# adria0/plonk-by-fingers

Measured on AMD Instinct MI355X. Metric: NTT elements/sec (Goldilocks, n=2^20 per GPU, natural order, bit-exact vs src/fft.rs), higher is better.
Workload: dtype u64 (Goldilocks p=2^64-2^32+1); 1 GPU; Goldilocks forward NTT, batch 32 x 2^20; n_per_gpu=1048576, n_global=1048576, batch=32, passes=default (2^20: 10,10)

## Files before the change

plonk-by-fingers_amd/csrc/internal.hpp:

```cpp
#pragma once
#include <hip/hip_runtime.h>
#include <stdint.h>
#include <cstdlib>
#include <map>
#include <memory>
#include <string>
#include <tuple>
#include <vector>
#include "field.hpp"

struct pbf_ctx;

namespace pbf {

typedef unsigned __int128 u128;
static const uint64_t GOLDILOCKS = 0xFFFFFFFF00000001ull;

enum FieldKind { FIELD_GOLDILOCKS = 0, FIELD_MOD32 = 1 };

void set_error(const std::string& s);

struct Options {
  std::map<std::string, std::string> kv;
  const char* get(const char* name) const {
    auto it = kv.find(name);
    return it == kv.end() ? nullptr : it->second.c_str();
  }
  long long num(const char* name, long long dflt) const {
    const char* v = get(name);
    return v && *v ? atoll(v) : dflt;
  }
};

int fail(int code, const std::string& s);

#define PBF_HIP(expr)                                                                        \
  do {                                                                                       \
    hipError_t e_ = (expr);                                                                  \
    if (e_ != hipSuccess)                                                                    \
      return ::pbf::fail(3 , std::string(#expr) + ": " + hipGetErrorString(e_)); \
  } while (0)

inline uint64_t hmul(uint64_t a, uint64_t b, uint64_t m) { return (uint64_t)(((u128)a * b) % m); }
inline uint64_t hpow(uint64_t a, uint64_t e, uint64_t m) {
  uint64_t r = 1 % m;
  while (e) {
    if (e & 1) r = hmul(r, a, m);
    a = hmul(a, a, m);
    e >>= 1;
  }
  return r;
}
bool hinv(uint64_t a, uint64_t m, uint64_t* out);

bool field_for(uint64_t m, FieldKind* kind, FieldArgs* fa);

struct DevBuf {
  void* p = nullptr;
  size_t bytes = 0;
  int ensure(size_t need);
  void release();
  ~DevBuf();
};

struct CosetTabs {
  uint64_t shift = 0, len = 0, stamp = 0;
  uint32_t bits = 0;
  DevBuf t0, t1;
  DevBuf tc_last;
};
constexpr size_t COSET_SHIFTS_PER_PLAN = 4;

struct NttPlan {
  uint64_t m = 0, omega = 0, n = 0;
  int inverse = 0;
  uint64_t root = 0;
  FieldKind kind = FIELD_GOLDILOCKS;
  FieldArgs fa{};
  uint32_t log_n = 0;
  uint64_t n_inv = 1;
  Options opts;
  std::vector<int> logr;
  int e64 = -1;
  std::vector<std::shared_ptr<DevBuf>> twpass;
  uint32_t tw_bits = 0;
  DevBuf tw0, tw1, small_tw;
  int twmax_log = 24;
  bool gl = false;
  std::vector<std::shared_ptr<DevBuf>> rtab;
  std::vector<std::shared_ptr<DevBuf>> tc;
  std::shared_ptr<DevBuf> tws_a, tws_b;
  int tws_w = 0;
  bool rg = false;
  mutable bool rg_built = false;
  mutable DevBuf rg_tc1, rg_t2;
  mutable DevBuf rg_tgc, rg_tgb;
  mutable std::vector<std::unique_ptr<CosetTabs>> coset;
  mutable uint64_t coset_clock = 0;
};

constexpr int GL_MAX_STREAMS = 8;
struct ForkSet {
  int device = 0;
  hipStream_t aux[GL_MAX_STREAMS] = {};
  hipEvent_t fork = nullptr, join[GL_MAX_STREAMS] = {};
  int ensure(int streams);
  ~ForkSet();
};

constexpr int MSM_TAIL_SLOTS = 3;
struct MsmTail {
  int device = 0;
  hipStream_t aux = nullptr;
  hipEvent_t ready[MSM_TAIL_SLOTS] = {}, done[MSM_TAIL_SLOTS] = {};
  bool used[MSM_TAIL_SLOTS] = {};
  int next = 0, last = -1;
  int ensure();
  ~MsmTail();
};

int make_plan(uint64_t m, uint64_t omega, uint64_t n, int inverse, NttPlan* p);
int run_plan(const NttPlan& p, const uint64_t* d_in, uint64_t* d_out, size_t batch, DevBuf& s0, DevBuf& s1,
             hipStream_t stream, ForkSet* fork = nullptr);
int run_plan_coset(const NttPlan& p, uint64_t shift, const uint64_t* d_in, size_t in_len, uint64_t* d_out,
                   size_t batch, DevBuf& s0, DevBuf& s1, hipStream_t stream, ForkSet* fork = nullptr);
int launch_pointwise_mul(FieldKind k, const FieldArgs& fa, const uint64_t* a, const uint64_t* b, uint64_t* c,
                         uint64_t count, hipStream_t s);
int launch_poly_eval(FieldKind k, const FieldArgs& fa, const uint64_t* d_coeffs, uint64_t n, const uint64_t* d_xs,
                     uint64_t nx, uint64_t* d_ys, DevBuf& partial, hipStream_t s);
struct TwoLevel {
  DevBuf t0, t1;
  uint64_t root = 0;
  uint32_t bits = 0;
};
int make_two_level(uint64_t m, uint64_t root, uint64_t n, TwoLevel* t);
int run_plan_split(const NttPlan& p, const uint64_t* d_in, uint64_t* d_send, size_t batch, uint32_t G, DevBuf& s0,
                   DevBuf& s1, DevBuf& s2, hipStream_t stream);
int launch_shard_combine(FieldKind k, const FieldArgs& fa, const TwoLevel& tl, uint32_t G, uint64_t rank,
                         const uint64_t* in, uint64_t* out, uint64_t nl, uint32_t batch, int inverse, hipStream_t s);
int launch_shard_unsplit(const uint64_t* recv, uint64_t* out, uint64_t nl, uint32_t batch, uint32_t G,
                         hipStream_t s);
int launch_fill_random(const FieldArgs& fa, FieldKind k, uint64_t seed, uint64_t* d_out, uint64_t count,
                       hipStream_t s);

int pairing_check_on_stream(pbf_ctx* ctx, const uint64_t* g1, const uint64_t* g2, size_t n, int* ok, hipStream_t s);

}

struct pbf_ctx {
  int device = 0;
  pbf::Options options;
  uint64_t serial = 0;
  hipStream_t stream = nullptr;
  hipStream_t user_stream = nullptr;
  std::map<std::tuple<uint64_t, uint64_t, uint64_t, int>, std::unique_ptr<pbf::NttPlan>> plans;
  pbf::DevBuf scratch0, scratch1, scratch2, io0, io1, io2, partial;
  pbf::ForkSet fork;
  struct FixedBase {
    bool valid = false;
    uint64_t n = 0;
    int c = 16;
    pbf::DevBuf table;
    pbf::DevBuf inf;
  } fixed_base;
  std::map<std::tuple<uint64_t, uint64_t, uint64_t>, std::unique_ptr<pbf::TwoLevel>> two_level;
  int roots(uint64_t m, uint64_t root, uint64_t n, pbf::TwoLevel** out);
  static hipStream_t pick(void* s) { return (hipStream_t)s; }
  hipStream_t host_stream() const { return user_stream ? user_stream : stream; }
  int plan(uint64_t m, uint64_t omega, uint64_t n, int inverse, pbf::NttPlan** out);
  std::map<std::string, std::unique_ptr<pbf::DevBuf>> named;
  pbf::DevBuf& buf(const std::string& name) {
    auto& b = named[name];
    if (!b) b.reset(new pbf::DevBuf());
    return *b;
  }
// ... 9 lines not shown
```

plonk-by-fingers_amd/csrc/ntt_gl.hpp:

```cpp
#pragma once
#include "ntt_kernels.hpp"

namespace pbf {

struct GlPassArgs {
  const uint64_t* in;
  uint64_t* out;
  const uint64_t* twpass;
  const uint64_t* tw0;
  const uint64_t* tw1;
  const uint64_t* tc;
  const uint64_t* tws_a;
  const uint64_t* tws_b;
  uint64_t n;
  uint32_t log_n;
  uint32_t log_ns;
  uint32_t tw_bits;
  uint32_t blocks_per_poly;
  uint32_t batch;
  uint32_t scaled;
  uint32_t out_split_log;
  uint32_t xcd_kmajor;
  uint64_t in_pitch, out_pitch;
  const uint64_t* post_tw;
  uint32_t skip_pass_tw;
  const uint64_t* cs_tab;
  const uint64_t* cs_tab1;
  uint32_t cs_bits;
  uint64_t cs_len;
};

__host__ __device__ constexpr bool gl_pow2_neg(int k) {
  const int raw = ((k % 192) + 192) % 192;
  return raw > 64 && raw <= 160;
}
template <int K>
__device__ __forceinline__ uint64_t gl_pow2_abs(uint64_t x) {
  constexpr int RAW = ((K % 192) + 192) % 192;
  if constexpr (RAW == 0) {
    return x;
  } else if constexpr (RAW > 160) {
    return gl_div_pow2<192 - RAW>(x);
  } else {
    using T = ShiftKind<RAW>;
    static_assert(T::NEG == gl_pow2_neg(K), "sign of 2^K");
    return apply_shift<Goldilocks, T>(x);
  }
}
template <int K>
__device__ __forceinline__ uint64_t gl_pow2(uint64_t x) {
  const uint64_t y = gl_pow2_abs<K>(x);
  if constexpr (gl_pow2_neg(K)) {
    const FieldArgs f{};
    return Goldilocks::sub(0, y, f);
  } else {
    return y;
  }
}

template <int E64, int Q1, int S2 = 1>
__device__ __forceinline__ void gl_stage_b_twiddle(uint64_t* v) {
  if constexpr (S2 < 16) {
    v[S2] = gl_pow2<(E64 * S2 * Q1) % 192>(v[S2]);
    gl_stage_b_twiddle<E64, Q1, S2 + 1>(v);
  }
}
template <int E64, int Q1, int S2 = 1>
__device__ __forceinline__ void gl_stage_b_twiddle_abs(uint64_t* v) {
  if constexpr (S2 < 16) {
    v[S2] = gl_pow2_abs<(E64 * S2 * Q1) % 192>(v[S2]);
    gl_stage_b_twiddle_abs<E64, Q1, S2 + 1>(v);
  }
}
__host__ __device__ constexpr unsigned gl_stage_b_negmask(int e64, int q1) {
  unsigned m = 0;
  for (int s2 = 1; s2 < 16; ++s2) m |= gl_pow2_neg((e64 * s2 * q1) % 192) ? 1u << s2 : 0u;
  return m;
}
constexpr int GL_B_LEVELS = 2;
template <int E64, int Q1>
__device__ __forceinline__ void gl_stage_b_head(uint64_t* v) {
  const FieldArgs f{};
  gl_stage_b_twiddle_abs<E64, Q1>(v);
  dft_reg_signed<Goldilocks, 4, sub_root_exp(E64, 4), gl_stage_b_negmask(E64, Q1), GL_B_LEVELS>(v, f);
}

template <int E64, int Q, int E = 1>
__device__ __forceinline__ void gl_post_twiddle_br(uint64_t* v) {
  if constexpr (E < 16) {
    v[bitrev_c(E, 4)] = gl_pow2<(E64 * E * Q) % 192>(v[bitrev_c(E, 4)]);
    gl_post_twiddle_br<E64, Q, E + 1>(v);
  }
}
template <int E64, int WV, int U = 0>
__device__ __forceinline__ void gl_rg3_c_shift(uint64_t* x) {
  if constexpr (U < 4) {
    constexpr int g = WV + 4 * U;
    x[U * 4 + 1] = gl_pow2<(E64 * g) % 192>(x[U * 4 + 1]);
    x[U * 4 + 2] = gl_pow2<(E64 * 2 * g) % 192>(x[U * 4 + 2]);
    x[U * 4 + 3] = gl_pow2<(E64 * 3 * g) % 192>(x[U * 4 + 3]);
    gl_rg3_c_shift<E64, WV, U + 1>(x);
  }
}

template <int LOGR, int TILE>
struct GlShape {
  static constexpr int R = 1 << LOGR;
  static constexpr int LOGC = LOGR - 6;
  static constexpr int C = 1 << LOGC;
  static constexpr int W = TILE / R;
  static constexpr int NT = TILE / 16;
  static constexpr int WPQ = NT / 256;
  static constexpr bool YX = W == 16 && C > 1;
  static constexpr int YP = (YX ? 64 : 65) * W;
  static constexpr int LDS = (C * YP > TILE) ? C * YP : TILE;
  static constexpr bool LDS32K = LDS * 8 <= 32768;
  static constexpr int NSUB_C = (64 * W) / NT;
  __host__ __device__ static constexpr int ysw(int k1) {
    return W <= 32 ? (k1 / (32 / W)) & (W - 1) : (k1 & 31);
  }
  __host__ __device__ static constexpr int yidx(int r2, int k1, int w) {
    return r2 * YP + (YX ? (k1 ^ (r2 & 1)) : k1) * W + (w ^ ysw(k1));
  }
};

__device__ __forceinline__ void gl_tile_coords(const GlPassArgs& a, uint32_t tile, uint32_t tiles, uint32_t* poly,
                                               uint32_t* kb) {
  if (a.xcd_kmajor == 1) {
    const uint32_t v = (tile & 7) * (tiles >> 3) + (tile >> 3);
    *kb = v / a.batch;
    *poly = v % a.batch;
  } else if (a.xcd_kmajor == 2) {
    const uint32_t v = (tile & 7) * (tiles >> 3) + (tile >> 3);
    *poly = v / a.blocks_per_poly;
    *kb = v % a.blocks_per_poly;
  } else {
    *poly = tile / a.blocks_per_poly;
    *kb = tile % a.blocks_per_poly;
  }
}

__device__ __forceinline__ uint64_t gl_cs_factor(const GlPassArgs& a, uint64_t i) {
  const FieldArgs f{};
  if (a.cs_tab1) return Goldilocks::mul(a.cs_tab[i & ((1ull << a.cs_bits) - 1)], a.cs_tab1[i >> a.cs_bits], f);
  return a.cs_tab[i];
}

constexpr int GL_STORES = 16;

template <int LOGR, int E64, bool FIRST, int TILE, int RG = 0, int CS = 0, int SP = 0>
__device__ __forceinline__ void gl_tile(const GlPassArgs& a, uint64_t* lds, uint32_t tile, uint32_t tiles, int t) {
  using Sh = GlShape<LOGR, TILE>;
  constexpr int C = Sh::C, LOGC = Sh::LOGC, W = Sh::W, NT = Sh::NT, YP = Sh::YP;
  (void)YP;
  static_assert(Sh::NSUB_C * C == GL_STORES, "stores per thread");
  static_assert(SP == 0 || (!FIRST && RG == 0 && CS == 0 && SP <= 2), "SP: second pass of a plain two-pass plan");
  static_assert(RG == 0 || (LOGR == 8 && TILE == 4096 && FIRST == (RG == 1)), "RG shape");
  static_assert(CS == 0 || (FIRST == (CS == 1) && (RG == 0 || RG == 2 * CS - 1)), "CS 1: first pass, CS 2: last pass");
  const FieldArgs f{};
  using G = Goldilocks;
  uint32_t poly, kb;
  gl_tile_coords(a, tile, tiles, &poly, &kb);
  const uint64_t j0 = (uint64_t)kb * W;
  const uint64_t* in = a.in + (uint64_t)poly * a.in_pitch;
  const uint64_t stride = a.n >> LOGR;

  uint64_t v[16];
  if constexpr (CS == 1) {
#pragma unroll
    for (int h = 0; h < 2; ++h) {
      uint64_t tw[8];
#pragma unroll
      for (int uu = 0; uu < 2; ++uu) {
        const int idx = t + NT * (2 * h + uu);
        const int w = idx % W, r2 = (idx / W) % C, s2 = idx / (C * W);
#pragma unroll
        for (int s1 = 0; s1 < 4; ++s1) {
          const uint64_t i = (j0 + w) + (uint64_t)(16 * C * s1 + C * s2 + r2) * stride;
          const bool on = i < a.cs_len;
          v[8 * h + uu * 4 + s1] = on ? in[i] : 0;
          tw[uu * 4 + s1] = on ? gl_cs_factor(a, i) : 0;
        }
      }
#pragma unroll
      for (int m = 0; m < 8; ++m) v[8 * h + m] = G::mul(v[8 * h + m], tw[m], f);
    }
  } else {
#pragma unroll
    for (int u = 0; u < 4; ++u) {
      const int idx = t + NT * u;
      const int w = idx % W, r2 = (idx / W) % C, s2 = idx / (C * W);
#pragma unroll
      for (int s1 = 0; s1 < 4; ++s1) {
        const int r = 16 * C * s1 + C * s2 + r2;
        v[u * 4 + s1] = in[(j0 + w) + (uint64_t)r * stride];
      }
    }
  }
  uint64_t t3[RG == 3 ? 2 : 1];
  if constexpr (RG == 3) {
    const int wave = t >> 6, q1 = wave / Sh::WPQ, rw = (wave % Sh::WPQ) * 64 + (t & 63);
    const int r2 = rw / W, w = rw % W;
    const uint64_t X = ((uint64_t)q1 << 16) + j0 + w;
    t3[0] = a.tws_a[((uint64_t)r2 << 18) + X];
    t3[1] = a.tws_b[X];
  }
  if constexpr (!FIRST && RG != 3 && SP == 0) if (!a.skip_pass_tw) {
    const uint64_t kmask = (1ull << a.log_ns) - 1;
#pragma unroll
    for (int h = 0; h < 2; ++h) {
      uint64_t tw[8];
#pragma unroll
      for (int uu = 0; uu < 2; ++uu) {
        const int u = 2 * h + uu;
        const int idx = t + NT * u;
        const int w = idx % W, r2 = (idx / W) % C, s2 = idx / (C * W);
        const uint64_t k = (j0 + w) & kmask;
#pragma unroll
        for (int s1 = 0; s1 < 4; ++s1) {
          const uint64_t r = (uint64_t)(16 * C * s1 + C * s2 + r2);
          if (a.twpass) {
            tw[uu * 4 + s1] = a.twpass[(r << a.log_ns) + k];
          } else if (a.tws_a) {
            tw[uu * 4 + s1] = G::mul(a.tws_b[(uint64_t)kb * Sh::R + r], a.tws_a[r * W + w], f);
          } else {
            const uint64_t e = ((r * k) << (a.log_n - a.log_ns - LOGR)) & (a.n - 1);
            tw[uu * 4 + s1] = G::mul(a.tw0[e & ((1ull << a.tw_bits) - 1)], a.tw1[e >> a.tw_bits], f);
          }
        }
      }
#pragma unroll
      for (int m = 0; m < 8; ++m) v[8 * h + m] = G::mul(v[8 * h + m], tw[m], f);
    }
  }
#pragma unroll
  for (int u = 0; u < 4; ++u) dft_reg<G, 2, sub_root_exp(E64, 2)>(v + u * 4, nullptr, f);
#pragma unroll
  for (int u = 0; u < 4; ++u) {
    const int idx = t + NT * u;
    const int s2 = idx / (C * W), rw = idx % (C * W);
#pragma unroll
    for (int q1 = 0; q1 < 4; ++q1) lds[(q1 * 16 + s2) * (C * W) + rw] = v[u * 4 + bitrev_c(q1, 2)];
  }
  __syncthreads();

  {
    const int wave = t >> 6;
    const int q1 = wave / Sh::WPQ;
    const int rw = (wave % Sh::WPQ) * 64 + (t & 63);
#pragma unroll
    for (int s2 = 0; s2 < 16; ++s2) v[s2] = lds[(q1 * 16 + s2) * (C * W) + rw];
    if constexpr (RG == 3) {
      uint64_t p = t3[0];
      const uint64_t d = t3[1];
#pragma unroll
      for (int s2 = 0; s2 < 16; ++s2) {
        v[s2] = G::mul(v[s2], p, f);
        if (s2 < 15) p = G::mul(p, d, f);
      }
      dft_reg<G, 4, sub_root_exp(E64, 4)>(v, nullptr, f);
    } else {
      switch (__builtin_amdgcn_readfirstlane(q1)) {
        case 1: gl_stage_b_head<E64, 1>(v); break;
        case 2: gl_stage_b_head<E64, 2>(v); break;
        case 3: gl_stage_b_head<E64, 3>(v); break;
        default: gl_stage_b_head<E64, 0>(v); break;
      }
      dft_reg_tail<G, 4, sub_root_exp(E64, 4), GL_B_LEVELS>(v, f);
    }
    __syncthreads();
    const int r2 = rw / W, w = rw % W;
#pragma unroll
    for (int q2 = 0; q2 < 16; ++q2) {
      const int k1 = q1 + 4 * q2;
      lds[Sh::yidx(r2, k1, w)] = v[bitrev_c(q2, 4)];
    }
  }
  __syncthreads();

  auto c_map = [&](int u, int* k1, int* w) {
    const int idx = t + NT * u;
    if constexpr (FIRST) {
      *k1 = idx & 63;
      *w = idx >> 6;
    } else {
      *k1 = idx / W;
      *w = idx % W;
    }
  };
  uint64_t x[Sh::NSUB_C * C];
#pragma unroll
  for (int u = 0; u < Sh::NSUB_C; ++u) {
    int k1, w;
    c_map(u, &k1, &w);
#pragma unroll
    for (int r2 = 0; r2 < C; ++r2) x[u * C + r2] = lds[Sh::yidx(r2, k1, w)];
  }
  if constexpr (RG == 3) {
    switch (__builtin_amdgcn_readfirstlane(t >> 6)) {
      case 0: gl_rg3_c_shift<E64, 0>(x); break;
      case 1: gl_rg3_c_shift<E64, 1>(x); break;
      case 2: gl_rg3_c_shift<E64, 2>(x); break;
      default: gl_rg3_c_shift<E64, 3>(x); break;
    }
  } else if constexpr (RG == 1) {
    const uint64_t* tc = a.tc + ((j0 >> 12) & 15) * 256;
#pragma unroll
    for (int u = 0; u < Sh::NSUB_C; ++u) {
      int k1, w;
      c_map(u, &k1, &w);
      uint64_t tw[C];
#pragma unroll
      for (int r2 = 0; r2 < C; ++r2) tw[r2] = tc[r2 * 64 + k1];
#pragma unroll
      for (int r2 = 0; r2 < C; ++r2) x[u * C + r2] = G::mul(x[u * C + r2], tw[r2], f);
    }
  } else {
    uint64_t tw[Sh::NSUB_C * C];
    const bool scaled = SP == 0 && a.scaled;
    const int r2lo = scaled ? 0 : 1;
#pragma unroll
    for (int u = 0; u < Sh::NSUB_C; ++u) {
      int k1, w;
      c_map(u, &k1, &w);
#pragma unroll
      for (int r2 = 0; r2 < C; ++r2) tw[u * C + r2] = (r2 >= r2lo) ? a.tc[r2 * 64 + k1] : 1;
    }
    if (scaled) {
#pragma unroll
      for (int m = 0; m < Sh::NSUB_C * C; ++m) x[m] = G::mul(x[m], tw[m], f);
    } else {
#pragma unroll
      for (int u = 0; u < Sh::NSUB_C; ++u)
#pragma unroll
        for (int r2 = 1; r2 < C; ++r2) x[u * C + r2] = G::mul(x[u * C + r2], tw[u * C + r2], f);
    }
  }
  if constexpr (C > 1) {
#pragma unroll
    for (int u = 0; u < Sh::NSUB_C; ++u) dft_reg<G, LOGC, sub_root_exp(E64, LOGC)>(x + u * C, nullptr, f);
  }

  if constexpr (FIRST) {
    uint64_t* o = a.out + (uint64_t)poly * a.out_pitch;
#pragma unroll
    for (int u = 0; u < Sh::NSUB_C; ++u) {
      int k1, w;
      c_map(u, &k1, &w);
      const uint64_t base = (j0 + w) << LOGR;
      if (a.post_tw) {
        uint64_t tw[C];
#pragma unroll
        for (int k2 = 0; k2 < C; ++k2) tw[k2] = a.post_tw[base + k1 + 64 * k2];
#pragma unroll
        for (int k2 = 0; k2 < C; ++k2) x[u * C + bitrev_c(k2, LOGC)] = G::mul(x[u * C + bitrev_c(k2, LOGC)], tw[k2], f);
      }
#pragma unroll
      for (int k2 = 0; k2 < C; ++k2) o[base + k1 + 64 * k2] = x[u * C + bitrev_c(k2, LOGC)];
    }
  } else {
    const uint32_t lns = SP == 2 ? (uint32_t)LOGR : a.log_ns;
    const uint64_t ns_mask = (1ull << lns) - 1;
    uint64_t* out = a.out + (uint64_t)poly * a.out_pitch;
    const uint32_t sl = SP != 0 ? 0u : a.out_split_log;
#pragma unroll
    for (int u = 0; u < Sh::NSUB_C; ++u) {
      int k1, w;
      c_map(u, &k1, &w);
      const uint64_t j = j0 + w;
      const uint64_t base = ((j >> lns) << (lns + LOGR)) + (j & ns_mask);
      if (sl == 0) {
        if constexpr (CS == 2) {
          uint64_t tw[C];
#pragma unroll
          for (int k2 = 0; k2 < C; ++k2) tw[k2] = gl_cs_factor(a, base + ((uint64_t)(k1 + 64 * k2) << lns));
#pragma unroll
          for (int k2 = 0; k2 < C; ++k2) x[u * C + bitrev_c(k2, LOGC)] = G::mul(x[u * C + bitrev_c(k2, LOGC)], tw[k2], f);
        }
#pragma unroll
        for (int k2 = 0; k2 < C; ++k2) out[base + ((uint64_t)(k1 + 64 * k2) << lns)] = x[u * C + bitrev_c(k2, LOGC)];
      } else {
        const uint64_t smask = (1ull << sl) - 1;
#pragma unroll
        for (int k2 = 0; k2 < C; ++k2) {
          const uint64_t kk = base + ((uint64_t)(k1 + 64 * k2) << lns);
          a.out[((((kk >> sl) * a.batch) + poly) << sl) + (kk & smask)] = x[u * C + bitrev_c(k2, LOGC)];
        }
      }
    }
  }
}

template <int LOGR, int TILE>
__device__ __forceinline__ void gl_shape_checks() {
  using Sh = GlShape<LOGR, TILE>;
  static_assert(LOGR >= 6 && LOGR <= 10, "radix 2^6 .. 2^10");
  static_assert(Sh::LDS * 8 <= (TILE > 8192 ? 160 : 80) * 1024, "LDS budget");
  static_assert(Sh::W >= 8 && Sh::WPQ >= 1, "tile shape");
}

template <int LOGR, int E64, bool FIRST, int TILE, int RG = 0, int CS = 0, int SP = 0>
__global__ void __launch_bounds__(TILE / 16)
__attribute__((amdgpu_waves_per_eu((FIRST || RG) && GlShape<LOGR, TILE>::LDS32K ? 5 : 4)))
ntt_gl_pass_kernel(GlPassArgs a) {
  gl_shape_checks<LOGR, TILE>();
  __shared__ __attribute__((aligned(16))) uint64_t lds[GlShape<LOGR, TILE>::LDS];
  const uint32_t tiles = a.blocks_per_poly * a.batch;
  gl_tile<LOGR, E64, FIRST, TILE, RG, CS, SP>(a, lds, blockIdx.x, tiles, threadIdx.x);
}

template <int E64>
__global__ void __launch_bounds__(256) __attribute__((amdgpu_waves_per_eu(4))) ntt_gl_rg2_kernel(GlPassArgs a) {
  constexpr int W = 16;
  __shared__ __attribute__((aligned(16))) uint64_t lds[16 * 16 * W];
  const FieldArgs f{};
  using G = Goldilocks;
  const uint32_t tiles = a.blocks_per_poly * a.batch;
  uint32_t poly, kb;
  gl_tile_coords(a, blockIdx.x, tiles, &poly, &kb);
  const int t = threadIdx.x, w = t % W, a1h = t / W;
  const uint64_t j0 = (uint64_t)kb * W, j = j0 + w;
  const uint32_t c = (uint32_t)(j0 >> 6) & 3, a1l = (uint32_t)(j0 >> 14) & 3;
  const uint64_t* in = a.in + (uint64_t)poly * a.in_pitch;
  const uint64_t stride = a.n >> 8;
  uint64_t v[16], tw[16];
#pragma unroll
// ... 32 lines not shown
```

plonk-by-fingers_amd/csrc/ntt_launch.hip:

```cpp
#include <cstdlib>
#include <cstring>
#include <mutex>
#include "internal.hpp"
#include "ntt_gl.hpp"

namespace pbf {

bool hinv(uint64_t a, uint64_t m, uint64_t* out) {
  __int128 s = 0, old_s = 1, r = m, old_r = a % m;
  while (r != 0) {
    __int128 q = old_r / r, t;
    t = old_r - q * r; old_r = r; r = t;
    t = old_s - q * s; old_s = s; s = t;
  }
  if (old_r != 1) return false;
  if (old_s < 0) old_s += m;
  *out = (uint64_t)old_s;
  return true;
}

bool field_for(uint64_t m, FieldKind* kind, FieldArgs* fa) {
  fa->m = m;
  fa->mu = 0;
  if (m == GOLDILOCKS) { *kind = FIELD_GOLDILOCKS; return true; }
  if (m >= 3 && m < (1ull << 32) && (m & 1)) {
    *kind = FIELD_MOD32;
    fa->mu = (uint64_t)(((u128)1 << 64) / m);
    return true;
  }
  return false;
}

int DevBuf::ensure(size_t need) {
  if (need <= bytes) return 0;
  if (p) (void)hipFree(p);
  p = nullptr;
  bytes = 0;
  hipError_t e = hipMalloc(&p, need);
  if (e != hipSuccess) { p = nullptr; return fail(3, std::string("hipMalloc: ") + hipGetErrorString(e)); }
  bytes = need;
  return 0;
}
void DevBuf::release() {
  if (p) (void)hipFree(p);
  p = nullptr;
  bytes = 0;
}
DevBuf::~DevBuf() { release(); }

static int upload(DevBuf& b, const std::vector<uint64_t>& v) {
  int rc = b.ensure(v.size() * 8);
  if (rc) return rc;
  PBF_HIP(hipMemcpy(b.p, v.data(), v.size() * 8, hipMemcpyHostToDevice));
  return 0;
}

typedef std::vector<uint64_t> Table;

static Table geometric(uint64_t c, uint64_t s, uint64_t count, uint64_t m) {
  Table t(count);
  uint64_t x = c % m;
  for (uint64_t i = 0; i < count; ++i) { t[i] = x; x = hmul(x, s, m); }
  return t;
}

static std::pair<Table, Table> two_level_tabs(uint64_t root, uint64_t len, uint32_t bits, uint64_t c, uint64_t m) {
  return {geometric(c, root, 1ull << bits, m),
          geometric(1, hpow(root, 1ull << bits, m), ((len - 1) >> bits) + 1, m)};
}

static Table stage_c_tab(uint64_t w_r, uint64_t C, uint64_t scale, uint64_t m) {
  Table tc(C * 64);
  for (uint64_t r2 = 0; r2 < C; ++r2)
    for (uint64_t k1 = 0; k1 < 64; ++k1) tc[r2 * 64 + k1] = hmul(hpow(w_r, r2 * k1, m), scale, m);
  return tc;
}

static Table pass_tab(uint64_t w_p, uint64_t R, uint64_t ns, uint64_t m) {
  Table t;
  t.reserve(R * ns);
  for (uint64_t r = 0; r < R; ++r) {
    const Table row = geometric(1, hpow(w_p, r, m), ns, m);
    t.insert(t.end(), row.begin(), row.end());
  }
  return t;
}

static std::pair<Table, Table> split_tabs(uint64_t w_p, uint64_t R, uint64_t W, uint64_t ns, uint64_t m) {
  Table ta = pass_tab(w_p, R, W, m), tb((ns / W) * R);
  for (uint64_t r = 0; r < R; ++r) {
    const Table col = geometric(1, hpow(w_p, r * W, m), ns / W, m);
    for (uint64_t kb = 0; kb < ns / W; ++kb) tb[kb * R + r] = col[kb];
  }
  return {ta, tb};
}

static std::vector<int> default_passes(uint32_t log_n, const Options& o) {
  const char* env = o.get("ntt.passes");
  if (env && *env) {
    std::vector<int> v;
    int sum = 0;
    for (const char* c = env; *c;) {
      int x = atoi(c);
      v.push_back(x);
      sum += x;
      while (*c && *c != ',') ++c;
      if (*c == ',') ++c;
    }
    bool ok = sum == (int)log_n;
    for (int x : v) ok = ok && x >= 6 && x <= 12;
    if (ok) return v;
  }
  int p = (log_n + 9) / 10;
  std::vector<int> v(p, log_n / p);
  for (int i = 0; i < (int)(log_n % p); ++i) v[i] += 1;
  return v;
}

static constexpr int gl_tile(int logr) { return logr >= 10 ? 8192 : 4096; }

int make_plan(uint64_t m, uint64_t omega, uint64_t n, int inverse, NttPlan* p) {
  if (!field_for(m, &p->kind, &p->fa)) return fail(5, "unsupported modulus");
  if (n == 0 || (n & (n - 1))) return fail(1, "n must be a power of two");
  if (n > (1ull << 32)) return fail(1, "n too large");
  if (omega >= m) return fail(1, "omega not canonical");
  uint32_t log_n = 0;
  while ((1ull << log_n) < n) ++log_n;
  if (n > 1) {
    if (hpow(omega, n, m) != 1 || hpow(omega, n / 2, m) == 1) return fail(1, "omega does not have order n");
  }
  p->m = m; p->omega = omega; p->n = n; p->inverse = inverse; p->log_n = log_n;
  p->root = omega;
  if (inverse) {
    if (!hinv(n % m, m, &p->n_inv)) return fail(2, "n has no inverse modulo M (fft.rs:73 unwrap)");
    if (!hinv(omega, m, &p->root)) return fail(1, "omega not invertible");
  }
  const uint64_t w = p->root;
  const long long tm = p->opts.num("ntt.twmax_log", 24);
  p->twmax_log = (int)(tm < 0 ? 0 : (tm > 30 ? 30 : tm));
  if (n <= 4096) return upload(p->small_tw, geometric(1, w, n, m));
  p->logr = default_passes(log_n, p->opts);
  p->tw_bits = (log_n + 1) / 2;
  p->e64 = -1;
  if (p->kind == FIELD_GOLDILOCKS) {
    const uint64_t w64 = hpow(w, n / 64, m);
    if (w64 == hpow(2, 39, m)) p->e64 = 39;
    else if (w64 == hpow(2, 153, m)) p->e64 = 153;
  }
  p->gl = p->e64 >= 0;
  for (int lr : p->logr) p->gl = p->gl && lr >= 6 && lr <= 10;
  p->rg = p->gl && log_n == 24 && p->logr == std::vector<int>{8, 8, 8} && p->opts.num("ntt.no_rg", 0) == 0;

  int rc;
  const auto tw = two_level_tabs(w, n, p->tw_bits, 1, m);
  if ((rc = upload(p->tw0, tw.first)) || (rc = upload(p->tw1, tw.second))) return rc;
  const size_t P = p->logr.size();
  uint64_t ns = 1;
  for (size_t i = 0; i < P; ++i) {
    const uint64_t R = 1ull << p->logr[i], w_p = hpow(w, n / (ns * R), m);
    p->twpass.push_back(std::make_shared<DevBuf>());
    if (ns > 1 && R * ns <= (1ull << p->twmax_log) && (rc = upload(*p->twpass[i], pass_tab(w_p, R, ns, m)))) return rc;
    const long long ts = p->opts.num("ntt.twsplit", -1);
    const uint64_t W = (uint64_t)gl_tile(p->logr[i]) >> p->logr[i];
    if (i + 1 == P && ns > 1 && p->e64 >= 0 && ts != 0 && p->logr[i] >= 6 && p->logr[i] <= 10 &&
        (!p->twpass[i]->p || ts == 1) && ns % W == 0) {
      if (ts == 1) p->twpass[i] = std::make_shared<DevBuf>();
      const auto ab = split_tabs(w_p, R, W, ns, m);
      p->tws_a = std::make_shared<DevBuf>();
      p->tws_b = std::make_shared<DevBuf>();
      if ((rc = upload(*p->tws_a, ab.first)) || (rc = upload(*p->tws_b, ab.second))) return rc;
      p->tws_w = (int)W;
    }
    ns *= R;
  }
  for (size_t i = 0; i < P; ++i) {
    const uint64_t R = 1ull << p->logr[i], w_r = hpow(w, n / R, m);
    auto b = std::make_shared<DevBuf>();
    if (p->gl) {
      rc = upload(*b, stage_c_tab(w_r, R / 64, (inverse && i + 1 == P) ? p->n_inv : 1, m));
      p->tc.push_back(b);
    } else {
      rc = upload(*b, geometric(1, w_r, R, m));
      p->rtab.push_back(b);
    }
    if (rc) return rc;
  }
  return 0;
}

template <class Fn>
static auto with_field(FieldKind k, Fn&& fn) {
  return k == FIELD_GOLDILOCKS ? fn(Goldilocks{}) : fn(Mod32{});
}

typedef void (*PassFn)(PassArgs);

static constexpr int cols_for(int logr) {
  return logr < 10 ? 16 : (logr == 10 ? 8 : (logr == 11 ? 8 : 4));
}

template <class F, int E>
static PassFn pass_fn_e(int logr) {
#define PBF_PASS(LR) \
  case LR: return ntt_pass_kernel<F, LR, cols_for(LR), ((cols_for(LR) << LR) >> NTT_LQ), E>;
  switch (logr) {
    PBF_PASS(6) PBF_PASS(7) PBF_PASS(8) PBF_PASS(9) PBF_PASS(10) PBF_PASS(11) PBF_PASS(12)
    default: return nullptr;
  }
#undef PBF_PASS
}

static PassFn pass_fn(FieldKind k, int e64, int logr) {
  if (k == FIELD_MOD32) return pass_fn_e<Mod32, -1>(logr);
  if (e64 == 39) return pass_fn_e<Goldilocks, 39>(logr);
  if (e64 == 153) return pass_fn_e<Goldilocks, 153>(logr);
  return pass_fn_e<Goldilocks, -1>(logr);
}

struct GlCoset {
  const CosetTabs* tabs;
  uint64_t in_len;
};

static int run_plan_impl(const NttPlan& p, const uint64_t* d_in, uint64_t* d_out, size_t batch, DevBuf& s0,
                         DevBuf& s1, hipStream_t stream, uint32_t split_log, ForkSet* fork = nullptr,
                         const GlCoset* cs = nullptr);

int run_plan(const NttPlan& p, const uint64_t* d_in, uint64_t* d_out, size_t batch, DevBuf& s0, DevBuf& s1,
             hipStream_t stream, ForkSet* fork) {
  return run_plan_impl(p, d_in, d_out, batch, s0, s1, stream, 0, fork);
}

__global__ void shard_split_kernel(const uint64_t* in, uint64_t* out, uint64_t s, uint64_t nl, uint32_t batch) {
  const uint64_t total = nl * batch;
  for (uint64_t id = (uint64_t)blockIdx.x * blockDim.x + threadIdx.x; id < total;
       id += (uint64_t)gridDim.x * blockDim.x) {
    const uint64_t b = id / nl, k = id % nl;
    out[((k / s) * batch + b) * s + (k % s)] = in[id];
  }
}

static uint64_t grid_for(uint64_t count) {
  uint64_t b = (count + 255) / 256;
  return b > 8192 ? 8192 : (b ? b : 1);
}

int run_plan_split(const NttPlan& p, const uint64_t* d_in, uint64_t* d_send, size_t batch, uint32_t G, DevBuf& s0,
                   DevBuf& s1, DevBuf& s2, hipStream_t stream) {
  const uint64_t S = p.n / G;
  uint32_t sl = 0;
  while ((1ull << sl) < S) ++sl;
  if (!p.logr.empty() && S >= 16 && p.logr.size() >= 2) return run_plan_impl(p, d_in, d_send, batch, s0, s1, stream, sl);
  int rc = s2.ensure(batch * p.n * 8);
  if (rc) return rc;
  if ((rc = run_plan_impl(p, d_in, (uint64_t*)s2.p, batch, s0, s1, stream, 0))) return rc;
  hipLaunchKernelGGL(shard_split_kernel, dim3(grid_for(p.n * batch)), dim3(256), 0, stream, (const uint64_t*)s2.p,
                     d_send, S, p.n, (uint32_t)batch);
  PBF_HIP(hipGetLastError());
  return 0;
}

int launch_shard_unsplit(const uint64_t* recv, uint64_t* out, uint64_t nl, uint32_t batch, uint32_t G,
                         hipStream_t s) {
  hipLaunchKernelGGL(shard_unsplit_kernel, dim3(grid_for(nl * batch)), dim3(256), 0, s, recv, out, nl / G, nl, batch,
                     G);
  PBF_HIP(hipGetLastError());
  return 0;
}

int make_two_level(uint64_t m, uint64_t root, uint64_t n, TwoLevel* t) {
  uint32_t log_n = 0;
  while ((1ull << log_n) < n) ++log_n;
  t->bits = (log_n + 1) / 2;
  t->root = root;
  const auto tw = two_level_tabs(root, n, t->bits, 1, m);
  int rc = upload(t->t0, tw.first);
  return rc ? rc : upload(t->t1, tw.second);
}

template <class F>
static int combine_typed(const FieldArgs& fa, const TwoLevel& tl, uint32_t G, uint64_t rank, const uint64_t* in,
                         uint64_t* out, uint64_t nl, uint32_t batch, int inverse, hipStream_t s) {
  CombineArgs a;
  a.recv = in; a.out = out;
  a.tw0 = (const uint64_t*)tl.t0.p; a.tw1 = (const uint64_t*)tl.t1.p; a.tw_bits = tl.bits;
  a.nl = nl; a.s = nl / G; a.rank = rank; a.n_mask = (uint64_t)G * nl - 1; a.batch = batch; a.f = fa;
  a.scale = 1;
  if (inverse) {
    uint64_t ginv;
    if (!hinv(G % fa.m, fa.m, &ginv)) return fail(2, "G has no inverse");
    a.scale = ginv;
  }
  for (int i = 0; i < 8; ++i) a.wg[i] = 0;
  const uint64_t wG = hpow(tl.root, nl, fa.m);
  uint64_t x = 1 % fa.m;
  for (uint32_t i = 0; i < G; ++i) { a.wg[i] = x; x = hmul(x, wG, fa.m); }
  const uint64_t total = (nl / G) * batch;
  void (*fn)(CombineArgs) = nullptr;
  switch (G) {
    case 2: fn = inverse ? shard_split_inv_kernel<F, 2> : shard_combine_kernel<F, 2>; break;
    case 4: fn = inverse ? shard_split_inv_kernel<F, 4> : shard_combine_kernel<F, 4>; break;
    case 8: fn = inverse ? shard_split_inv_kernel<F, 8> : shard_combine_kernel<F, 8>; break;
    default: return fail(1, "world size must be 2, 4 or 8");
  }
  hipLaunchKernelGGL(fn, dim3(grid_for(total)), dim3(256), 0, s, a);
  PBF_HIP(hipGetLastError());
  return 0;
}

int launch_shard_combine(FieldKind k, const FieldArgs& fa, const TwoLevel& tl, uint32_t G, uint64_t rank,
                         const uint64_t* in, uint64_t* out, uint64_t nl, uint32_t batch, int inverse, hipStream_t s) {
  return with_field(k, [&](auto F) {
    return combine_typed<decltype(F)>(fa, tl, G, rank, in, out, nl, batch, inverse, s);
  });
}

typedef void (*GlPassFn)(GlPassArgs);

struct GlPassDesc {
  int logr;
  bool first;
  int rg;
  int cs;
  int sp;
};

static bool two_pass_tw(const NttPlan& p, uint32_t split_log) {
  return p.logr.size() == 2 && split_log == 0 && p.twpass[1]->p;
}

static GlPassDesc gl_pass_desc(const NttPlan& p, size_t i, bool coset, uint32_t split_log) {
  const size_t P = p.logr.size();
  GlPassDesc d{p.logr[i], i == 0, 0, 0, 0};
  if (p.rg && P == 3 && split_log == 0) d.rg = (int)i + 1;
  if (coset && !p.inverse && i == 0) d.cs = 1;
  if (coset && p.inverse && i == P - 1) d.cs = 2;
  if (two_pass_tw(p, split_log) && i == 1 && !coset && !p.inverse && p.e64 == 39 && d.logr == 10)
    d.sp = p.logr[0] == 10 ? 2 : 1;
  return d;
}

template <int E, int LR>
static GlPassFn gl_kernel_lr(const GlPassDesc& d) {
  constexpr int T = gl_tile(LR);
  if (d.first) return d.cs ? ntt_gl_pass_kernel<LR, E, true, T, 0, 1> : ntt_gl_pass_kernel<LR, E, true, T>;
  return d.cs ? ntt_gl_pass_kernel<LR, E, false, T, 0, 2> : ntt_gl_pass_kernel<LR, E, false, T>;
}

template <int E>
static GlPassFn gl_kernel_e(const GlPassDesc& d) {
  if (d.rg == 1) return d.cs ? ntt_gl_pass_kernel<8, E, true, 4096, 1, 1> : ntt_gl_pass_kernel<8, E, true, 4096, 1>;
  if (d.rg == 2) return ntt_gl_rg2_kernel<E>;
  if (d.rg == 3) return d.cs ? ntt_gl_pass_kernel<8, E, false, 4096, 3, 2> : ntt_gl_pass_kernel<8, E, false, 4096, 3>;
  if constexpr (E == 39) {
    if (d.sp == 1) return ntt_gl_pass_kernel<10, E, false, 8192, 0, 0, 1>;
    if (d.sp == 2) return ntt_gl_pass_kernel<10, E, false, 8192, 0, 0, 2>;
  }
  switch (d.logr) {
    case 6: return gl_kernel_lr<E, 6>(d);
    case 7: return gl_kernel_lr<E, 7>(d);
    case 8: return gl_kernel_lr<E, 8>(d);
    case 9: return gl_kernel_lr<E, 9>(d);
    case 10: return gl_kernel_lr<E, 10>(d);
    default: return nullptr;
  }
}

static GlPassFn gl_kernel(const GlPassDesc& d, int e64) {
  return e64 == 39 ? gl_kernel_e<39>(d) : gl_kernel_e<153>(d);
}

static int run_gl_group(const NttPlan& p, const uint64_t* d_in, uint64_t* d_out, size_t batch, DevBuf& s0,
                        DevBuf& s1, hipStream_t stream, uint32_t split_log, size_t soff = 0,
                        const GlCoset* cs = nullptr);

int ForkSet::ensure(int streams) {
  if (streams > GL_MAX_STREAMS) streams = GL_MAX_STREAMS;
  const unsigned flags = hipEventDisableTiming | hipEventDisableSystemFence;
  if (streams > 1 && !fork) PBF_HIP(hipEventCreateWithFlags(&fork, flags));
  for (int i = 1; i < streams; ++i) {
    if (!aux[i]) PBF_HIP(hipStreamCreateWithFlags(&aux[i], hipStreamNonBlocking));
    if (!join[i]) PBF_HIP(hipEventCreateWithFlags(&join[i], flags));
  }
  return 0;
}

ForkSet::~ForkSet() {
  (void)hipSetDevice(device);
  for (int i = 1; i < GL_MAX_STREAMS; ++i) {
    if (aux[i]) {
      (void)hipStreamSynchronize(aux[i]);
      (void)hipStreamDestroy(aux[i]);
    }
    if (join[i]) (void)hipEventDestroy(join[i]);
  }
  if (fork) (void)hipEventDestroy(fork);
}

static void gl_schedule(const NttPlan& p, size_t batch, uint32_t split_log, const ForkSet* fork, size_t* G, int* ns) {
  const long long go = p.opts.num("ntt.group", -1);
  *G = go >= 0 ? (size_t)go : (batch >= 8 ? 4 : batch);
  if (split_log != 0 || *G >= batch) *G = 0;
  *ns = (int)p.opts.num("ntt.streams", 2);
  *ns = *ns < 1 ? 1 : (*ns > GL_MAX_STREAMS ? GL_MAX_STREAMS : *ns);
  if (!fork || *G == 0) *ns = 1;
}

static size_t gl_scratch_polys(const NttPlan& p, size_t batch, uint32_t split_log, const ForkSet* fork) {
  size_t G;
  int ns;
  gl_schedule(p, batch, split_log, fork, &G, &ns);
  return (G == 0 || G * ns > batch) ? batch : G * ns;
}

static int run_gl_passes(const NttPlan& p, const uint64_t* d_in, uint64_t* d_out, size_t batch, DevBuf& s0,
                         DevBuf& s1, hipStream_t stream, uint32_t split_log, ForkSet* fork, const GlCoset* cs) {
  size_t G;
  int ns;
  gl_schedule(p, batch, split_log, fork, &G, &ns);
  if (G == 0) return run_gl_group(p, d_in, d_out, batch, s0, s1, stream, split_log, 0, cs);
  const size_t in_pitch = (cs && !p.inverse) ? cs->in_len : p.n;
  hipStream_t sts[GL_MAX_STREAMS];
  sts[0] = stream;
  if (ns > 1) {
    int rc = fork->ensure(ns);
    if (rc) return rc;
    for (int i = 1; i < ns; ++i) sts[i] = fork->aux[i];
    PBF_HIP(hipEventRecord(fork->fork, stream));
    for (int i = 1; i < ns; ++i) PBF_HIP(hipStreamWaitEvent(sts[i], fork->fork, 0));
  }
  int gi = 0;
  for (size_t g0 = 0; g0 < batch; g0 += G, ++gi) {
    const size_t b = batch - g0 < G ? batch - g0 : G;
    const int rc = run_gl_group(p, d_in + g0 * in_pitch, d_out + g0 * p.n, b, s0, s1, sts[gi % ns], 0,
                                (size_t)(gi % ns) * G * p.n, cs);
    if (rc) return rc;
  }
  for (int i = 1; i < ns; ++i) {
    PBF_HIP(hipEventRecord(fork->join[i], sts[i]));
    PBF_HIP(hipStreamWaitEvent(stream, fork->join[i], 0));
  }
  return 0;
}

static int ensure_rg_tables(const NttPlan& p) {
  if (p.rg_built) return 0;
  const uint64_t m = p.m, n = p.n;
  const uint64_t w = p.root;
  int rc;
  const uint64_t w4096 = hpow(w, n / 4096, m);
  std::vector<uint64_t> tc1(4096);
  for (uint64_t a2l = 0; a2l < 16; ++a2l)
    for (uint64_t r2 = 0; r2 < 4; ++r2)
      for (uint64_t k1 = 0; k1 < 64; ++k1)
        tc1[a2l * 256 + r2 * 64 + k1] = hpow(w4096, ((a2l + 16 * r2) * k1) % 4096, m);
  const Table t2 = pass_tab(hpow(w, 64, m), 64, 4096, m);
  const uint64_t scale = p.inverse ? p.n_inv : 1;
  std::vector<uint64_t> tgc(4ull << 18), tgb(1ull << 18);
  {
    const uint64_t w4 = hpow(w, 4, m);
    uint64_t x1 = 1, x4 = 1;
    for (uint64_t X = 0; X < (1ull << 18); ++X) {
      tgb[X] = x4;
      uint64_t c = scale;
      for (uint64_t r2 = 0; r2 < 4; ++r2) {
        tgc[(r2 << 18) + X] = c;
        c = hmul(c, x1, m);
      }
      x1 = hmul(x1, w, m);
      x4 = hmul(x4, w4, m);
    }
  }
  if ((rc = upload(p.rg_tc1, tc1)) || (rc = upload(p.rg_t2, t2)) || (rc = upload(p.rg_tgc, tgc)) ||
      (rc = upload(p.rg_tgb, tgb)))
    return rc;
  p.rg_built = true;
  return 0;
}

static GlPassArgs gl_pass_args(const NttPlan& p, size_t i, const GlPassDesc& d, uint32_t log_ns, const uint64_t* in,
                               uint64_t* out, size_t batch, uint32_t split_log, const GlCoset* cs) {
  const bool last = i == p.logr.size() - 1;
  const uint64_t W = (uint64_t)gl_tile(d.logr) >> d.logr;
  GlPassArgs a;
  a.in = in;
  a.out = out;
  a.in_pitch = a.out_pitch = p.n;
  a.twpass = (const uint64_t*)p.twpass[i]->p;
  a.tw0 = (const uint64_t*)p.tw0.p;
  a.tw1 = (const uint64_t*)p.tw1.p;
  a.tc = (const uint64_t*)p.tc[i]->p;
  const bool tws = !a.twpass && last && p.tws_a && (uint64_t)p.tws_w == W;
  a.tws_a = tws ? (const uint64_t*)p.tws_a->p : nullptr;
  a.tws_b = tws ? (const uint64_t*)p.tws_b->p : nullptr;
  a.n = p.n;
  a.log_n = p.log_n;
  a.log_ns = log_ns;
  a.tw_bits = p.tw_bits;
  a.blocks_per_poly = (uint32_t)((p.n >> d.logr) / W);
  a.batch = (uint32_t)batch;
  a.scaled = (p.inverse && last) ? 1 : 0;
  a.out_split_log = last ? split_log : 0;
  const uint64_t tiles = (uint64_t)a.blocks_per_poly * batch;
  a.xcd_kmajor = (log_ns > 0 && batch > 1 && tiles % 8 == 0) ? 1 : 0;
  a.post_tw = nullptr;
  a.skip_pass_tw = 0;
  if (two_pass_tw(p, split_log)) {
    if (i == 0) a.post_tw = (const uint64_t*)p.twpass[1]->p;
    else a.skip_pass_tw = 1;
  }
  if (a.post_tw && batch > 1 && tiles % 8 == 0) a.xcd_kmajor = 1;
  a.cs_tab = a.cs_tab1 = nullptr;
  a.cs_bits = 0;
  a.cs_len = 0;
  if (d.cs) {
    a.cs_tab = (const uint64_t*)cs->tabs->t0.p;
    a.cs_tab1 = (const uint64_t*)cs->tabs->t1.p;
    a.cs_bits = cs->tabs->bits;
    if (d.cs == 1) {
      a.cs_len = cs->in_len;
      a.in_pitch = cs->in_len;
    } else if (!d.rg) {
      a.tc = (const uint64_t*)cs->tabs->tc_last.p;
      a.scaled = 0;
    }
  }
  if (d.rg) {
    if (d.rg == 1) a.tc = (const uint64_t*)p.rg_tc1.p;
    if (d.rg == 2) a.twpass = (const uint64_t*)p.rg_t2.p;
    if (d.rg == 3) {
      a.twpass = nullptr;
      a.tws_a = (const uint64_t*)p.rg_tgc.p;
      a.tws_b = (const uint64_t*)p.rg_tgb.p;
    }
    if (tiles % 8 == 0) a.xcd_kmajor = 2;
  }
  return a;
}

static int run_gl_group(const NttPlan& p, const uint64_t* d_in, uint64_t* d_out, size_t batch, DevBuf& s0,
                        DevBuf& s1, hipStream_t stream, uint32_t split_log, size_t soff, const GlCoset* cs) {
  const size_t P = p.logr.size();
  if (cs && (split_log != 0 || P < 2)) return fail(1, "coset transform: unsupported plan");
  if (gl_pass_desc(p, 0, cs != nullptr, split_log).rg) {
    const int rc = ensure_rg_tables(p);
    if (rc) return rc;
  }
  uint32_t log_ns = 0;
  for (size_t i = 0; i < P; ++i) {
    const GlPassDesc d = gl_pass_desc(p, i, cs != nullptr, split_log);
    const GlPassFn fn = gl_kernel(d, p.e64);
    if (!fn) return fail(1, "no Goldilocks pass kernel for this radix");
    const int tile = gl_tile(d.logr);
    if ((p.n >> d.logr) % (tile >> d.logr)) return fail(1, "transform too small for the pass tile");
    const uint64_t* in = (i == 0) ? d_in : (const uint64_t*)(((i - 1) & 1) ? s1.p : s0.p) + soff;
    uint64_t* out = (i == P - 1) ? d_out : (uint64_t*)((i & 1) ? s1.p : s0.p) + soff;
    const GlPassArgs a = gl_pass_args(p, i, d, log_ns, in, out, batch, split_log, cs);
    const uint64_t tiles = (uint64_t)a.blocks_per_poly * batch;
    if (tiles > 0x7fffffffull) return fail(1, "batch too large");
    hipLaunchKernelGGL(fn, dim3((uint32_t)tiles), dim3(tile / 16), 0, stream, a);
    PBF_HIP(hipGetLastError());
    log_ns += d.logr;
  }
  return 0;
}

static int run_plan_impl(const NttPlan& p, const uint64_t* d_in, uint64_t* d_out, size_t batch, DevBuf& s0,
                         DevBuf& s1, hipStream_t stream, uint32_t split_log, ForkSet* fork, const GlCoset* cs) {
  if (batch == 0) return 0;
  if (p.n == 1) {
    if (d_in != d_out) PBF_HIP(hipMemcpyAsync(d_out, d_in, batch * 8, hipMemcpyDeviceToDevice, stream));
    return 0;
  }
  if (p.logr.empty()) {
    with_field(p.kind, [&](auto F) {
      hipLaunchKernelGGL(ntt_small_kernel<decltype(F)>, dim3(batch), dim3(256), 0, stream, d_in, d_out,
                         (const uint64_t*)p.small_tw.p, p.log_n, p.n_inv, (uint32_t)p.inverse, p.fa);
    });
    PBF_HIP(hipGetLastError());
    return 0;
  }
  const size_t P = p.logr.size();
  const size_t bytes = (p.gl ? gl_scratch_polys(p, batch, split_log, fork) : batch) * p.n * 8;
  int rc = s0.ensure(bytes);
  if (!rc && P > 2) rc = s1.ensure(bytes);
  if (rc) return rc;
  uint32_t log_ns = 0;
  if (p.gl) return run_gl_passes(p, d_in, d_out, batch, s0, s1, stream, split_log, fork, cs);
  if (cs) return fail(1, "coset transform: not a Goldilocks standard-root plan");
  for (size_t i = 0; i < P; ++i) {
    const int lr = p.logr[i];
    const PassFn fn = pass_fn(p.kind, p.e64, lr);
    if (!fn) return fail(1, "no kernel for this radix");
    const int W = cols_for(lr);
    PassArgs a;
    a.in = (i == 0) ? d_in : (const uint64_t*)(((i - 1) & 1) ? s1.p : s0.p);
    a.out = (i == P - 1) ? d_out : (uint64_t*)((i & 1) ? s1.p : s0.p);
    a.tw0 = (const uint64_t*)p.tw0.p;
    a.tw1 = (const uint64_t*)p.tw1.p;
    a.rtab = (const uint64_t*)p.rtab[i]->p;
    a.twpass = (const uint64_t*)p.twpass[i]->p;
    a.n = p.n;
    a.n_inv = p.n_inv;
    a.log_n = p.log_n;
    a.log_ns = log_ns;
    a.tw_bits = p.tw_bits;
    a.blocks_per_poly = (uint32_t)((p.n >> lr) / W);
    a.scale = (p.inverse && i == P - 1) ? 1 : 0;
    a.out_split_log = (i == P - 1) ? split_log : 0;
    a.batch = (uint32_t)batch;
    a.f = p.fa;
    const int nt = (W << lr) >> NTT_LQ;
    const uint64_t blocks = (uint64_t)a.blocks_per_poly * batch;
    if (blocks > 0x7fffffffull) return fail(1, "batch too large");
    const uint32_t grid = (uint32_t)blocks;
    a.xcd_kmajor = (log_ns > 0 && batch > 1 && grid % 8 == 0) ? 1 : 0;
    hipLaunchKernelGGL(fn, dim3(grid), dim3(nt), 0, stream, a);
    PBF_HIP(hipGetLastError());
    log_ns += lr;
  }
  return 0;
}

static uint32_t log2_ceil(uint64_t x) {
  uint32_t l = 0;
  while ((1ull << l) < x) ++l;
  return l;
}

static int coset_tabs(const NttPlan& p, uint64_t shift, uint64_t len, const CosetTabs** out) {
  const uint64_t m = p.m;
  CosetTabs* t = nullptr;
  for (auto& c : p.coset)
    if (c->shift == shift) t = c.get();
  if (t && t->len >= len) {
    t->stamp = ++p.coset_clock;
    *out = t;
    return 0;
  }
  if (!t) {
    if (p.coset.size() >= COSET_SHIFTS_PER_PLAN) {
      size_t old = 0;
      for (size_t i = 1; i < p.coset.size(); ++i)
        if (p.coset[i]->stamp < p.coset[old]->stamp) old = i;
      p.coset.erase(p.coset.begin() + old);
    }
    p.coset.emplace_back(new CosetTabs());
    t = p.coset.back().get();
    t->shift = shift;
  } else {
    PBF_HIP(hipDeviceSynchronize());
  }
  t->len = 0;
  uint64_t s = shift, c = 1 % m;
  if (p.inverse) {
    if (!hinv(shift, m, &s)) return fail(1, "shift has no inverse");
    if (p.gl && !p.rg) c = p.n_inv;
  }
  int rc;
  if (len <= (1ull << p.twmax_log)) {
    t->bits = 0;
    t->t1.release();
    if ((rc = upload(t->t0, geometric(c, s, len, m)))) return rc;
  } else {
    t->bits = (log2_ceil(len) + 1) / 2;
    const auto tw = two_level_tabs(s, len, t->bits, c, m);
// ... 164 lines not shown
```

Baseline: 108.8 billion elements/s.

## Use tile-major blocked intermediate layout between passes of the 10,10 Goldilocks NTT

For the forward two-pass 10,10 Goldilocks plan, the first pass now writes its twiddled output into a tile-major blocked scratch layout (pitch 8192 per block). The second pass reads that layout with contiguous 128-bit vector loads and stores to LDS in vector form. The twiddle table is also pre-laid out in matching blocked order. The goal is to replace strided global accesses between passes with coalesced, contiguous ones. In exchange it adds a new twiddle table, slightly larger scratch, and new kernel instantiations.

```diff
diff --git a/plonk-by-fingers_amd/csrc/internal.hpp b/plonk-by-fingers_amd/csrc/internal.hpp
--- a/plonk-by-fingers_amd/csrc/internal.hpp
+++ b/plonk-by-fingers_amd/csrc/internal.hpp
@@ -91,6 +91,7 @@
   std::vector<std::shared_ptr<DevBuf>> tc;
   std::shared_ptr<DevBuf> tws_a, tws_b;
   int tws_w = 0;
+  DevBuf post_blk;
   bool rg = false;
   mutable bool rg_built = false;
   mutable DevBuf rg_tc1, rg_t2;
diff --git a/plonk-by-fingers_amd/csrc/ntt_gl.hpp b/plonk-by-fingers_amd/csrc/ntt_gl.hpp
--- a/plonk-by-fingers_amd/csrc/ntt_gl.hpp
+++ b/plonk-by-fingers_amd/csrc/ntt_gl.hpp
@@ -24,6 +24,7 @@
   uint64_t in_pitch, out_pitch;
   const uint64_t* post_tw;
   uint32_t skip_pass_tw;
+  uint64_t blk_pitch;
   const uint64_t* cs_tab;
   const uint64_t* cs_tab1;
   uint32_t cs_bits;
@@ -148,13 +149,18 @@
 
 constexpr int GL_STORES = 16;
 
+constexpr uint64_t GL_BLK_PITCH = 8192;
+static_assert(GL_BLK_PITCH >= 8192 && GL_BLK_PITCH % 2 == 0, "block pitch");
+typedef uint64_t gl_u64x2 __attribute__((ext_vector_type(2)));
+
 template <int LOGR, int E64, bool FIRST, int TILE, int RG = 0, int CS = 0, int SP = 0>
 __device__ __forceinline__ void gl_tile(const GlPassArgs& a, uint64_t* lds, uint32_t tile, uint32_t tiles, int t) {
   using Sh = GlShape<LOGR, TILE>;
   constexpr int C = Sh::C, LOGC = Sh::LOGC, W = Sh::W, NT = Sh::NT, YP = Sh::YP;
   (void)YP;
   static_assert(Sh::NSUB_C * C == GL_STORES, "stores per thread");
-  static_assert(SP == 0 || (!FIRST && RG == 0 && CS == 0 && SP <= 2), "SP: second pass of a plain two-pass plan");
+  static_assert(SP == 0 || ((!FIRST || SP == 2) && RG == 0 && CS == 0 && SP <= 2), "SP: plain two-pass plan");
+  static_assert(SP != 2 || (LOGR == 10 && TILE == 8192), "SP 2: the 10,10 plan");
   static_assert(RG == 0 || (LOGR == 8 && TILE == 4096 && FIRST == (RG == 1)), "RG shape");
   static_assert(CS == 0 || (FIRST == (CS == 1) && (RG == 0 || RG == 2 * CS - 1)), "CS 1: first pass, CS 2: last pass");
   const FieldArgs f{};
@@ -164,9 +170,18 @@
   const uint64_t j0 = (uint64_t)kb * W;
   const uint64_t* in = a.in + (uint64_t)poly * a.in_pitch;
   const uint64_t stride = a.n >> LOGR;
+  constexpr bool BLK_IN = SP == 2 && !FIRST, BLK_OUT = SP == 2 && FIRST;
 
   uint64_t v[16];
-  if constexpr (CS == 1) {
+  if constexpr (BLK_IN) {
+    const gl_u64x2* blk = (const gl_u64x2*)(in + (uint64_t)kb * a.blk_pitch) + t;
+#pragma unroll
+    for (int up = 0; up < 8; ++up) {
+      const gl_u64x2 e = blk[512 * up];
+      v[(2 * (up & 1)) * 4 + (up >> 1)] = e.x;
+      v[(2 * (up & 1) + 1) * 4 + (up >> 1)] = e.y;
+    }
+  } else if constexpr (CS == 1) {
 #pragma unroll
     for (int h = 0; h < 2; ++h) {
       uint64_t tw[8];
@@ -235,12 +250,26 @@
   }
 #pragma unroll
   for (int u = 0; u < 4; ++u) dft_reg<G, 2, sub_root_exp(E64, 2)>(v + u * 4, nullptr, f);
-#pragma unroll
-  for (int u = 0; u < 4; ++u) {
-    const int idx = t + NT * u;
-    const int s2 = idx / (C * W), rw = idx % (C * W);
-#pragma unroll
-    for (int q1 = 0; q1 < 4; ++q1) lds[(q1 * 16 + s2) * (C * W) + rw] = v[u * 4 + bitrev_c(q1, 2)];
+  if constexpr (BLK_IN) {
+#pragma unroll
+    for (int h = 0; h < 2; ++h) {
+      const int s2 = 8 * h + (t >> 6);
+#pragma unroll
+      for (int q1 = 0; q1 < 4; ++q1) {
+        gl_u64x2 e;
+        e.x = v[(2 * h) * 4 + bitrev_c(q1, 2)];
+        e.y = v[(2 * h + 1) * 4 + bitrev_c(q1, 2)];
+        *(gl_u64x2*)(lds + (q1 * 16 + s2) * (C * W) + 2 * (t & 63)) = e;
+      }
+    }
+  } else {
+#pragma unroll
+    for (int u = 0; u < 4; ++u) {
+      const int idx = t + NT * u;
+      const int s2 = idx / (C * W), rw = idx % (C * W);
+#pragma unroll
+      for (int q1 = 0; q1 < 4; ++q1) lds[(q1 * 16 + s2) * (C * W) + rw] = v[u * 4 + bitrev_c(q1, 2)];
+    }
   }
   __syncthreads();
 
@@ -280,7 +309,10 @@
 
   auto c_map = [&](int u, int* k1, int* w) {
     const int idx = t + NT * u;
-    if constexpr (FIRST) {
+    if constexpr (BLK_OUT) {
+      *k1 = 8 * (t >> 6) + (t & 7);
+      *w = (t >> 3) & 7;
+    } else if constexpr (FIRST) {
       *k1 = idx & 63;
       *w = idx >> 6;
     } else {
@@ -341,7 +373,20 @@
     for (int u = 0; u < Sh::NSUB_C; ++u) dft_reg<G, LOGC, sub_root_exp(E64, LOGC)>(x + u * C, nullptr, f);
   }
 
-  if constexpr (FIRST) {
+  if constexpr (BLK_OUT) {
+    static_assert(Sh::NSUB_C == 1 && W == 8, "tile-major stores: one sub-DFT per thread");
+    const uint64_t base = (uint64_t)__builtin_amdgcn_readfirstlane(t >> 6) * a.blk_pitch + j0 * W;
+    const uint32_t lane = t & 63;
+    const uint64_t* ptw = a.post_tw + base;
+    uint64_t* o = a.out + (uint64_t)poly * a.out_pitch + base;
+    uint64_t tw[C];
+#pragma unroll
+    for (int k2 = 0; k2 < C; ++k2) tw[k2] = ptw[(uint64_t)(8 * k2) * a.blk_pitch + lane];
+#pragma unroll
+    for (int k2 = 0; k2 < C; ++k2) x[bitrev_c(k2, LOGC)] = G::mul(x[bitrev_c(k2, LOGC)], tw[k2], f);
+#pragma unroll
+    for (int k2 = 0; k2 < C; ++k2) o[(uint64_t)(8 * k2) * a.blk_pitch + lane] = x[bitrev_c(k2, LOGC)];
+  } else if constexpr (FIRST) {
     uint64_t* o = a.out + (uint64_t)poly * a.out_pitch;
 #pragma unroll
     for (int u = 0; u < Sh::NSUB_C; ++u) {
diff --git a/plonk-by-fingers_amd/csrc/ntt_launch.hip b/plonk-by-fingers_amd/csrc/ntt_launch.hip
--- a/plonk-by-fingers_amd/csrc/ntt_launch.hip
+++ b/plonk-by-fingers_amd/csrc/ntt_launch.hip
@@ -82,6 +82,15 @@
   for (uint64_t r = 0; r < R; ++r) {
     const Table row = geometric(1, hpow(w_p, r, m), ns, m);
     t.insert(t.end(), row.begin(), row.end());
+  }
+  return t;
+}
+
+static Table pass_tab_blocked(uint64_t w, uint64_t pitch, uint64_t m) {
+  Table t(128 * pitch, 0);
+  for (uint64_t k = 0; k < 1024; ++k) {
+    const Table col = geometric(1, hpow(w, k, m), 1024, m);
+    for (uint64_t j = 0; j < 1024; ++j) t[(k >> 3) * pitch + j * 8 + (k & 7)] = col[j];
   }
   return t;
 }
@@ -173,6 +182,9 @@
     }
     ns *= R;
   }
+  if (p->gl && !inverse && p->e64 == 39 && p->logr == std::vector<int>{10, 10} && p->twpass[1]->p &&
+      (rc = upload(p->post_blk, pass_tab_blocked(w, GL_BLK_PITCH, m))))
+    return rc;
   for (size_t i = 0; i < P; ++i) {
     const uint64_t R = 1ull << p->logr[i], w_r = hpow(w, n / R, m);
     auto b = std::make_shared<DevBuf>();
@@ -329,14 +341,22 @@
   return p.logr.size() == 2 && split_log == 0 && p.twpass[1]->p;
 }
 
+static bool gl_blocked(const NttPlan& p, bool coset, uint32_t split_log) {
+  return two_pass_tw(p, split_log) && !coset && p.post_blk.p != nullptr;
+}
+
+static uint64_t gl_scratch_pitch(const NttPlan& p, bool coset, uint32_t split_log) {
+  return gl_blocked(p, coset, split_log) ? 128 * GL_BLK_PITCH : p.n;
+}
+
 static GlPassDesc gl_pass_desc(const NttPlan& p, size_t i, bool coset, uint32_t split_log) {
   const size_t P = p.logr.size();
   GlPassDesc d{p.logr[i], i == 0, 0, 0, 0};
   if (p.rg && P == 3 && split_log == 0) d.rg = (int)i + 1;
   if (coset && !p.inverse && i == 0) d.cs = 1;
   if (coset && p.inverse && i == P - 1) d.cs = 2;
-  if (two_pass_tw(p, split_log) && i == 1 && !coset && !p.inverse && p.e64 == 39 && d.logr == 10)
-    d.sp = p.logr[0] == 10 ? 2 : 1;
+  if (gl_blocked(p, coset, split_log)) d.sp = 2;
+  else if (two_pass_tw(p, split_log) && i == 1 && !coset && !p.inverse && p.e64 == 39 && d.logr == 10) d.sp = 1;
   return d;
 }
 
@@ -354,7 +374,7 @@
   if (d.rg == 3) return d.cs ? ntt_gl_pass_kernel<8, E, false, 4096, 3, 2> : ntt_gl_pass_kernel<8, E, false, 4096, 3>;
   if constexpr (E == 39) {
     if (d.sp == 1) return ntt_gl_pass_kernel<10, E, false, 8192, 0, 0, 1>;
-    if (d.sp == 2) return ntt_gl_pass_kernel<10, E, false, 8192, 0, 0, 2>;
+    if (d.sp == 2) return d.first ? ntt_gl_pass_kernel<10, E, true, 8192, 0, 0, 2> : ntt_gl_pass_kernel<10, E, false, 8192, 0, 0, 2>;
   }
   switch (d.logr) {
     case 6: return gl_kernel_lr<E, 6>(d);
@@ -433,7 +453,7 @@
   for (size_t g0 = 0; g0 < batch; g0 += G, ++gi) {
     const size_t b = batch - g0 < G ? batch - g0 : G;
     const int rc = run_gl_group(p, d_in + g0 * in_pitch, d_out + g0 * p.n, b, s0, s1, sts[gi % ns], 0,
-                                (size_t)(gi % ns) * G * p.n, cs);
+                                (size_t)(gi % ns) * G * gl_scratch_pitch(p, cs != nullptr, split_log), cs);
     if (rc) return rc;
   }
   for (int i = 1; i < ns; ++i) {
@@ -510,6 +530,17 @@
     else a.skip_pass_tw = 1;
   }
   if (a.post_tw && batch > 1 && tiles % 8 == 0) a.xcd_kmajor = 1;
+  a.blk_pitch = 0;
+  if (d.sp == 2) {
+    a.blk_pitch = GL_BLK_PITCH;
+    if (i == 0) {
+      a.post_tw = (const uint64_t*)p.post_blk.p;
+      a.out_pitch = 128 * GL_BLK_PITCH;
+    } else {
+      a.in_pitch = 128 * GL_BLK_PITCH;
+      a.xcd_kmajor = 0;
+    }
+  }
   a.cs_tab = a.cs_tab1 = nullptr;
   a.cs_bits = 0;
   a.cs_len = 0;
@@ -581,7 +612,8 @@
     return 0;
   }
   const size_t P = p.logr.size();
-  const size_t bytes = (p.gl ? gl_scratch_polys(p, batch, split_log, fork) : batch) * p.n * 8;
+  const size_t bytes = p.gl ? gl_scratch_polys(p, batch, split_log, fork) * gl_scratch_pitch(p, cs != nullptr, split_log) * 8
+                            : batch * p.n * 8;
   int rc = s0.ensure(bytes);
   if (!rc && P > 2) rc = s1.ensure(bytes);
   if (rc) return rc;
```

After: 110.7 billion elements/s, median of 6. 1.02x the previous value.
